# OCR-D/ocrd_keraslm

Measured on AMD Instinct MI355X. Metric: chars/sec training (stacked-LSTM forward+backward+Adam), higher is better.
Workload: dtype bf16; 1 GPU; cfg2: depth=2 width=512 length=256 V=256 1 context, stateful training, 3072 streams/GPU, synthetic 10M-char corpus (SURVEY.md 8d); streams_per_gpu=3072, global_batch=3072, seq_len=256, parallelism=dp1

## Files before the change

ocrd_keraslm_amd/csrc/api.hip:

```cpp
#include <hip/hip_runtime.h>
#include <stdio.h>
#include <stdlib.h>
#include <string.h>
#include <time.h>

#include <functional>
#include <utility>

#include <vector>

#include "kl_common.h"
#include "kl_kernels.h"

namespace {

inline size_t align_up(size_t x, size_t a) { return (x + a - 1) / a * a; }
inline int round_up_i(int x, int a) { return (x + a - 1) / a * a; }

struct Carver {
  unsigned char* base;
  size_t off = 0;
  explicit Carver(void* b) : base(reinterpret_cast<unsigned char*>(b)) {}
  template <typename T>
  T* take(size_t count) {
// ... 23 lines not shown
  unsigned* scan_flags = nullptr;
};

struct WindowWs {
  float* P1;
  std::vector<void*> H;
  std::vector<float*> C;
  float* logits;
  float* rowstat;
  int *s_idx, *s_ctx, *s_tgt;
  int* ids_tm = nullptr;
  int scan2_rows = 0;
  bool scan2_bwd = false;
  float *s_masks, *s_probs;
  unsigned *scan_cnt, *scan_status;
  float* reg_scratch;
  std::vector<bf16_t*> G, dZ, Hd;
  std::vector<bf16_t*> Cb;
  std::vector<bf16_t*> Xhi, Xlo;
  std::vector<bf16_t*> HTf, HdT;
  bool ht_ready = false;
  bool km_plan = false;
  bf16_t *dZT, *HT, *dlogits, *dlogitsT, *OHT, *dEKT_bf, *dEK_bf;
  std::vector<bf16_t*> OHC;
  float *dH, *dEKT;
  std::vector<float*> dc0, dc1, dCtxKT;
};

}

struct kl_handle {
  kl_config cfg;
  int Vp;
  size_t n_params;
  std::vector<size_t> off_K, off_U, off_b, off_Ctx;
  size_t off_E;
  float* params = nullptr;
  void* derived_ws = nullptr;
  size_t derived_bytes = 0;
  Derived d;
  int precision = 0;
  struct GraphKey {
    int kind, B, T, flags, precision;
    const void *states, *loss_acc, *ws, *grads;
    int layout = 0;
    bool operator==(const GraphKey& o) const {
// ... 35 lines not shown
  int inc_small_min = KL_SMALL_STEP_N;
  bool scan2 = true;
  int scan2_rows = 0;
  int scan2_pf = -1;
  bool scan2_bf16 = true;
  bool logits_ws = true;
  bool proj_ws = true;
  bool w128 = true;
  bool w128_tables = true;
  bool w128_multi = true;
  bool w128_fuse = true;
  int w128_min = 1;
  bool fwd8 = true;
  bool fwd8_all = false;
  bool fwd8_tab = true;
  bool fwd8_ls = true;
  bool fwd8_local = true;
  int fwd8_pf = -1;
  bool rt_local = true;
  bool regtile = true;
  bool scan2_flags = true;
  bool flags_zeroed = false;
  bool fuse_wg = true;
  int scan2_pfb = -1;
  int wide_fwd_min = 96;
  double trace_flops[2] = {0.0, 0.0};
  bool trace_on = false;
  std::vector<std::pair<hipEvent_t, hipEvent_t>> trace_ev[2];
  size_t trace_used[2] = {0, 0};
  bool trace_open[2] = {false, false};
  bool trace_persistent[2] = {false, false};
  const char* trace_name[2] = {"lstm_fwd_step_kernel", "lstm_bwd_step_kernel"};
  void trace_begin(int kind, hipStream_t s) {
    if (!trace_on) return;
    if (trace_used[kind] == trace_ev[kind].size()) {
      hipEvent_t a, b;
      if (hipEventCreate(&a) != hipSuccess || hipEventCreate(&b) != hipSuccess) { trace_on = false; return; }
      trace_ev[kind].emplace_back(a, b);
    }
    (void)hipEventRecord(trace_ev[kind][trace_used[kind]].first, s);
    trace_open[kind] = true;
  }
  void trace_end(int kind, hipStream_t s) {
    if (!trace_on || !trace_open[kind]) return;
    trace_open[kind] = false;
    (void)hipEventRecord(trace_ev[kind][trace_used[kind]].second, s);
// ... 132 lines not shown
  if (training) {
    o.G.assign(L, nullptr); o.dZ.assign(L, nullptr); o.Hd.assign(L, nullptr); o.Cb.assign(L, nullptr);
    o.dc0.assign(L, nullptr); o.dc1.assign(L, nullptr);
    for (size_t l = 0; l < L; ++l) {
      o.G[l] = cv.take<bf16_t>(BT * 4 * W);
      o.dZ[l] = cv.take<bf16_t>(BT * 4 * W);
      o.Hd[l] = l > 0 ? cv.take<bf16_t>(BT * W) : nullptr;
      o.Cb[l] = cv.take<bf16_t>((BT + B) * W);
      o.dc0[l] = cv.take<float>((size_t)B * W);
      o.dc1[l] = cv.take<float>((size_t)B * W);
    }
    o.dZT = cv.take<bf16_t>(4 * W * BTp);
    o.HT = cv.take<bf16_t>(W * BTp);
    o.ids_tm = cv.take<int>((BT + B) * 2);
    o.HTf.assign(L, nullptr); o.HdT.assign(L, nullptr);
    if ((B & 7) == 0) {
      for (size_t l = 0; l < L; ++l) {
        o.HTf[l] = cv.take<bf16_t>(W * (BT + B));
        o.HdT[l] = l > 0 ? cv.take<bf16_t>(W * BT) : nullptr;
      }
    }
    o.dlogits = cv.take<bf16_t>(BT * Vp);
    o.dlogitsT = cv.take<bf16_t>(Vp * BTp);
    o.OHT = cv.take<bf16_t>(Vp * BTp);
    o.OHC.assign(c.n_ctx, nullptr);
    o.dCtxKT.assign(c.n_ctx, nullptr);
    for (int n = 0; n < c.n_ctx; ++n) {
      o.OHC[n] = cv.take<bf16_t>((size_t)c.ctx_vocab * BTp);
      o.dCtxKT[n] = cv.take<float>(4 * W * (size_t)c.ctx_vocab);
    }
    o.dH = cv.take<float>(BT * W);
    o.dEKT = cv.take<float>(4 * W * Vp);
    o.dEKT_bf = cv.take<bf16_t>(4 * W * Vp);
    o.dEK_bf = cv.take<bf16_t>(Vp * 4 * W);
  }
  return align_up(cv.off, 256);
}

#define KL_TRY(expr)            \
  do {                          \
    int _e = (expr);            \
    if (_e != 0) return _e;     \
  } while (0)

int hip_ok(hipError_t e) { return e == hipSuccess ? 0 : KL_ERR_LAUNCH; }

int prepare_impl(kl_handle* h, int precision, hipStream_t s) {
  const kl_config& c = h->cfg;
  const int W = c.width, V = c.voc_size, Vp = h->Vp;
  const float* P = h->params;
  Derived& d = h->d;
  const bool split = precision == KL_PREC_SPLIT;
  if (!h->flags_zeroed) {
    hipStreamCaptureStatus cap = hipStreamCaptureStatusNone;
    if (hipStreamIsCapturing(s, &cap) == hipSuccess && cap == hipStreamCaptureStatusNone) {
      KL_TRY(kl_zero_async(d.scan_flags, (size_t)(KL_SCAN_FLAGS + 64) * sizeof(unsigned), s));
      h->flags_zeroed = true;
    }
  }
  const float* E = P + h->off_E;
// ... 129 lines not shown
      KlScanFwdWide a;
      memset(&a, 0, sizeof(a));
      a.B = B; a.T = T; a.W = W;
      a.UT = d.UT_hi[l];
      const bool v2 = w.scan2_rows != 0;
      const bool f8_tab = v2 && l == 0 && h->fwd8 && h->fwd8_tab && !h->fwd8_all && d.comb != nullptr && c.n_ctx == 1 && w.scan2_rows == 32 &&
                          h->scan2_bf16 && h->sentinel_roll && T >= 3 && h->fwd8_ls;
      const bool f8 = v2 && h->fwd8 && w.scan2_rows == 32 && h->scan2_bf16 && h->sentinel_roll && T >= 3 &&
                      (l > 0 || c.n_ctx > 1 || h->fwd8_all || f8_tab);
      if (l > 0) {
        const bool masked_in = masks != nullptr && (l - 1) > 0;
        const bf16_t* X = masked_in ? w.Hd[l - 1] : (const bf16_t*)w.H[l - 1] + BW;
        int pe = KL_ERR_SHAPE;
        if (v2 && h->scan2_bf16 && h->proj_ws)
          pe = kl_launch_proj_ws(X, d.KTp[l], d.bp[l], reinterpret_cast<bf16_t*>(w.P1), (long)B * T, W, w.scan_status, s);
        if (pe == KL_ERR_SHAPE)
          pe = kl_launch_gemm_tn(X, v2 ? d.KTp[l] : d.KT_hi[l], w.P1, v2 ? d.bp[l] : P + h->off_b[l], B * T, 4 * W, W, W, W, 4 * W,
                                 v2 && h->scan2_bf16 ? 1 : 0, 1, 1.f, s);
        KL_TRY(pe);
        a.P = w.P1;
        a.p_bf16 = v2 && h->scan2_bf16 ? 1 : 0;
      } else if (f8_tab) {
        KL_TRY(kl_launch_comb_table(d.EKp, d.CtxKp[0], c.voc_size, c.ctx_vocab, 4 * W, d.comb, s));
        KL_TRY(kl_launch_rows_tm(idx, ctx, c.n_ctx, B, T, c.ctx_vocab, w.ids_tm, s));
        a.P = reinterpret_cast<const float*>(d.comb);
        a.p_bf16 = 1;
        a.ids_tm = w.ids_tm;
        a.V = c.voc_size; a.ctx_vocab = c.ctx_vocab;
      } else if (v2 && (c.n_ctx > 1 || f8)) {
        KL_TRY(kl_launch_p_gather_il(d.EKp, d.CtxKp.data(), c.n_ctx, idx, ctx, B, T, W, c.voc_size, c.ctx_vocab,
                                     reinterpret_cast<bf16_t*>(w.P1), s));
        a.P = w.P1;
        a.p_bf16 = 1;
      } else if (v2) {
        KL_TRY(kl_launch_ids_tm(idx, ctx, c.n_ctx, B, T, W, c.voc_size, c.ctx_vocab, w.ids_tm, s));
        a.EK = d.EKp;
        a.CtxK[0] = c.n_ctx > 0 ? d.CtxKp[0] : nullptr;
        a.n_ctx = c.n_ctx;
        a.ids_tm = w.ids_tm;
        a.V = c.voc_size; a.ctx_vocab = c.ctx_vocab;
      } else {
        a.EK = d.EK;
        for (int n = 0; n < c.n_ctx; ++n) a.CtxK[n] = d.CtxK[n];
        a.n_ctx = c.n_ctx;
        a.idx = idx; a.ctx = ctx;
        a.bias = P + h->off_b[0];
      }
// ... 519 lines not shown
  const char* env8t = getenv("KL_W128_TABLES");
  if (env8t) h->w128_tables = atoi(env8t) != 0;
  const char* env8mm = getenv("KL_W128_MULTI");
  if (env8mm) h->w128_multi = atoi(env8mm) != 0;
  const char* env8q = getenv("KL_W128_MIN");
  if (env8q) h->w128_min = atoi(env8q);
  const char* env8m = getenv("KL_FWD8");
  if (env8m) { h->fwd8 = atoi(env8m) != 0; h->fwd8_all = atoi(env8m) == 2; }
  const char* env8r = getenv("KL_FWD8_LS");
  if (env8r) h->fwd8_ls = atoi(env8r) != 0;
  const char* env8n = getenv("KL_FWD8_LOCAL");
  if (env8n) h->fwd8_local = atoi(env8n) != 0;
  const char* env8o = getenv("KL_FWD8_PF");
  if (env8o) h->fwd8_pf = atoi(env8o);
  const char* env8l = getenv("KL_RT_LOCAL");
  if (env8l) h->rt_local = atoi(env8l) != 0;
  const char* env8k = getenv("KL_REGTILE");
  if (env8k) h->regtile = atoi(env8k) != 0;
  const char* env8g = getenv("KL_SCAN2_FLAGS");
  if (env8g) h->scan2_flags = atoi(env8g) != 0;
  h->flags_zeroed = false;
  const char* env8f = getenv("KL_FUSE_WG");
  if (env8f) h->fuse_wg = atoi(env8f) != 0;
  const char* env8d = getenv("KL_SCAN2_PFB");
  if (env8d) h->scan2_pfb = atoi(env8d);
  const char* env5 = getenv("KL_WIDE_FWD_MIN");
  if (env5) h->wide_fwd_min = atoi(env5);
  return kl_zero_page_ready();
}

int kl_prepare(kl_handle* h, int precision, void* stream) {
  if (!h) return KL_ERR_ARG;
  if (!h->params) return KL_ERR_STATE;
  if (precision != KL_PREC_BF16 && precision != KL_PREC_SPLIT) return KL_ERR_ARG;
  return prepare_impl(h, precision, (hipStream_t)stream);
}

size_t kl_window_workspace_bytes(const kl_handle* h, int B, int T, int training) {
  if (!h || B < 1 || T < 1) return 0;
  return carve_window(h, nullptr, B, T, training, nullptr);
}

static int forward_window_body(kl_handle* h, int B, int T, const int32_t* idx, const int32_t* ctx, const int32_t* tgt,
                      float* states, float* probs, float* loss_acc, void* ws, size_t ws_bytes, void* stream) {
  if (!h || !idx || !states || !ws || B < 1 || T < 1) return KL_ERR_ARG;
  if (h->cfg.n_ctx > 0 && !ctx) return KL_ERR_ARG;
// ... 122 lines not shown
    } else if (dz_km) {
      KL_TRY(kl_launch_gemm_an(w.dZ[l], (const bf16_t*)w.H[l], grads + h->off_U[l], 4 * W, W, BT, 4 * W, W, 4 * W, 1, s, 1));
    } else if (w.ht_ready) {
      KL_TRY(kl_launch_gemm_tn(w.HTf[l], w.dZT, grads + h->off_U[l], nullptr, W, 4 * W, BT, ldtf, BTp, 4 * W, 2, ksplit, 1.f, s));
    } else {
      KL_TRY(kl_launch_transpose_bf16((const bf16_t*)w.H[l], W, w.HT, BTp, BT, W, s));
      KL_TRY(kl_launch_gemm_tn(w.HT, w.dZT, grads + h->off_U[l], nullptr, W, 4 * W, BTp, BTp, BTp, 4 * W, 2, ksplit, 1.f, s));
    }
    if (!db_done) KL_TRY(kl_launch_colsum_bf16(w.dZ[l], 4 * W, BT, 4 * W, grads + h->off_b[l], s));
    if (l > 0) {
      const bool masked_in = masks != nullptr && (l - 1) > 0;
      const bf16_t* X = masked_in ? w.Hd[l - 1] : (const bf16_t*)w.H[l - 1] + BW;
      if (pair_uk) {
      } else if (dz_km) {
        KL_TRY(kl_launch_gemm_an(w.dZ[l], X, grads + h->off_K[l], 4 * W, W, BT, 4 * W, W, 4 * W, 1, s, 1));
      } else if (w.ht_ready) {
        const bf16_t* XT = masked_in ? w.HdT[l - 1] : w.HTf[l - 1] + B;
        KL_TRY(kl_launch_gemm_tn(XT, w.dZT, grads + h->off_K[l], nullptr, W, 4 * W, BT, masked_in ? (long)BT : ldtf, BTp, 4 * W, 2, ksplit, 1.f, s));
      } else {
        KL_TRY(kl_launch_transpose_bf16(X, W, w.HT, BTp, BT, W, s));
        KL_TRY(kl_launch_gemm_tn(w.HT, w.dZT, grads + h->off_K[l], nullptr, W, 4 * W, BTp, BTp, BTp, 4 * W, 2, ksplit, 1.f, s));
      }
    } else {
      if (kl_launch_onehot_dense(idx, B, T, Vp, 0, 1, w.OHT, BTp, s) == KL_ERR_SHAPE) {
        KL_TRY(kl_zero_async(w.OHT, (size_t)Vp * BTp * sizeof(bf16_t), s));
        KL_TRY(kl_launch_onehot_t(idx, B, T, V, 0, 1, w.OHT, BTp, s));
      }
      KL_TRY(kl_zero_async(w.dEKT, (size_t)4 * W * Vp * sizeof(float), s));
      bool pair_ctx = dz_km && h->fuse_wg && c.n_ctx >= 1 && (Vp % 128) == 0 &&
                      kl_gemm_an_applicable(4 * W, Vp + c.ctx_vocab, BT, 4 * W);
      if (pair_ctx) {
        if (kl_launch_onehot_dense(ctx, B, T, c.ctx_vocab, 0, c.n_ctx, w.OHC[0], BTp, s) == KL_ERR_SHAPE) {
          KL_TRY(kl_zero_async(w.OHC[0], (size_t)c.ctx_vocab * BTp * sizeof(bf16_t), s));
          KL_TRY(kl_launch_onehot_t(ctx, B, T, c.ctx_vocab, 0, c.n_ctx, w.OHC[0], BTp, s));
        }
        KL_TRY(kl_zero_async(w.dCtxKT[0], (size_t)4 * W * c.ctx_vocab * sizeof(float), s));
        const int pe = kl_launch_gemm_an2(w.dZ[l], w.OHT, w.dEKT, 4 * W, Vp, BT, 4 * W, BTp, Vp, 0,
                                          w.OHC[0], w.dCtxKT[0], c.ctx_vocab, BTp, c.ctx_vocab, 0, s, 0);
        if (pe == KL_ERR_SHAPE) pair_ctx = false;
        else KL_TRY(pe);
      }
      if (pair_ctx) {
      } else if (dz_km) KL_TRY(kl_launch_gemm_an(w.dZ[l], w.OHT, w.dEKT, 4 * W, Vp, BT, 4 * W, BTp, Vp, 0, s));
      else KL_TRY(kl_launch_gemm_tn(w.dZT, w.OHT, w.dEKT, nullptr, 4 * W, Vp, BTp, BTp, BTp, Vp, 2, ksplit, 1.f, s));
      KL_TRY(kl_launch_f32_to_bf16_t(w.dEKT, Vp, 4 * W, Vp, w.dEKT_bf, nullptr, Vp, 0, s));
      KL_TRY(kl_launch_f32_to_bf16_t(w.dEKT, Vp, 4 * W, Vp, w.dEK_bf, nullptr, 4 * W, 1, s));
      KL_TRY(kl_launch_gemm_tn(d.ET, w.dEKT_bf, grads + h->off_K[0], nullptr, W, 4 * W, Vp, Vp, Vp, 4 * W, 0, 1, 1.f, s));
      KL_TRY(kl_launch_gemm_tn(w.dEK_bf, d.Kn[0], grads + h->off_E, nullptr, V, W, 4 * W, 4 * W, 4 * W, W, 2, 1, 1.f, s));
      for (int n = 0; n < c.n_ctx; ++n) {
        if (!(pair_ctx && n == 0)) {
          if (kl_launch_onehot_dense(ctx, B, T, c.ctx_vocab, n, c.n_ctx, w.OHC[n], BTp, s) == KL_ERR_SHAPE) {
            KL_TRY(kl_zero_async(w.OHC[n], (size_t)c.ctx_vocab * BTp * sizeof(bf16_t), s));
            KL_TRY(kl_launch_onehot_t(ctx, B, T, c.ctx_vocab, n, c.n_ctx, w.OHC[n], BTp, s));
          }
          KL_TRY(kl_zero_async(w.dCtxKT[n], (size_t)4 * W * c.ctx_vocab * sizeof(float), s));
          if (dz_km) KL_TRY(kl_launch_gemm_an(w.dZ[l], w.OHC[n], w.dCtxKT[n], 4 * W, c.ctx_vocab, BT, 4 * W, BTp, c.ctx_vocab, 0, s));
          else KL_TRY(kl_launch_gemm_tn(w.dZT, w.OHC[n], w.dCtxKT[n], nullptr, 4 * W, c.ctx_vocab, BTp, BTp, BTp,
                                        c.ctx_vocab, 2, ksplit, 1.f, s));
        }
        const size_t krow = (size_t)(W + n * c.ctx_dim) * 4 * W;
        KL_TRY(kl_launch_ctx_grads(P + h->off_Ctx[n], P + h->off_K[0] + krow, 4 * W, c.ctx_vocab, c.ctx_dim,
                                   w.dCtxKT[n], c.ctx_vocab, 4 * W, grads + h->off_K[0] + krow, 4 * W,
                                   grads + h->off_Ctx[n], s));
      }
    }
      return 0;
  };
  bool bscanned = false;
  const int n_rb_all = (B + 15) / 16, nug = W / 16;
  const bool thin_fits = (n_rb_all + 512 / nug - 1) / (512 / nug) <= (W == 1024 ? 8 : 4) &&
                         (long)T * B * 4 * W * 2 <= 0xfffffff0L;
  const bool wide_fits = h->wide_bwd && kl_scan_bwd_wide_applicable(B, T, W) && BTp == BT && (B & 7) == 0;
  const bool seq128 = h->scan_enabled && h->seq_bwd && h->w128 && B >= h->w128_min && kl_scan_w128_applicable(B, T, W) && !w.scan2_bwd;
// ... 720 lines not shown
```

ocrd_keraslm_amd/csrc/elementwise.hip:

```cpp
#include <string.h>

#include "kl_common.h"
#include "kl_kernels.h"

namespace {

struct CtxTabs { const float* t[8]; };

__global__ void embed_gather_kernel(const float* __restrict__ E, CtxTabs tabs, int n_ctx, int ctx_dim, int W,
                                    const int* __restrict__ idx, const int* __restrict__ ctx, int B, int T,
                                    bf16_t* __restrict__ X, long ldx, int Dp) {
  const int chunks = Dp >> 3;
  const long total = (long)B * T * chunks;
  for (long e = blockIdx.x * (long)blockDim.x + threadIdx.x; e < total; e += (long)gridDim.x * blockDim.x) {
    const int c = (int)(e % chunks);
    const long row = e / chunks;
    const int b = (int)(row % B), t = (int)(row / B);
    const int id = idx[(long)b * T + t];
    frag16 o;
#pragma unroll
    for (int j = 0; j < 8; ++j) {
      const int d = c * 8 + j;
      float v = 0.f;
      if (d < W) {
// ... 453 lines not shown
    gx = max(gx, (jobs[j].cols + 63) / 64);
    gy = max(gy, (all.job[j].rows_pad + 63) / 64);
  }
  hipLaunchKernelGGL(f32_to_bf16_jobs_kernel, dim3(gx, gy, n), dim3(256), 0, stream, all);
  return ok();
}

__global__ void comb_table_kernel(const float* __restrict__ A, const float* __restrict__ B, int R2, int N8, bf16_t* __restrict__ out, long total) {
  for (long e = blockIdx.x * (long)blockDim.x + threadIdx.x; e < total; e += (long)gridDim.x * blockDim.x) {
    const int j = (int)(e % N8);
    const long row = e / N8;
    const int c = (int)(row % R2), v = (int)(row / R2);
    const float4* pa = reinterpret_cast<const float4*>(A + ((long)v * N8 + j) * 8);
    const float4* pb = reinterpret_cast<const float4*>(B + ((long)c * N8 + j) * 8);
    const float4 a0 = pa[0], a1 = pa[1], b0 = pb[0], b1 = pb[1];
    uint4 o;
    o.x = (unsigned)f2bf(a0.x + b0.x) | ((unsigned)f2bf(a0.y + b0.y) << 16);
    o.y = (unsigned)f2bf(a0.z + b0.z) | ((unsigned)f2bf(a0.w + b0.w) << 16);
    o.z = (unsigned)f2bf(a1.x + b1.x) | ((unsigned)f2bf(a1.y + b1.y) << 16);
    o.w = (unsigned)f2bf(a1.z + b1.z) | ((unsigned)f2bf(a1.w + b1.w) << 16);
    reinterpret_cast<uint4*>(out)[e] = o;
  }
}
__global__ void rows_tm_kernel(const int* __restrict__ idx, const int* __restrict__ ctx, int n_ctx, int Bn, int T, int R2, int* __restrict__ out) {
  const long total = (long)Bn * T;
  for (long e = blockIdx.x * (long)blockDim.x + threadIdx.x; e < total; e += (long)gridDim.x * blockDim.x) {
    const int b = (int)(e % Bn), t = (int)(e / Bn);
    const long src = (long)b * T + t;
    out[e] = idx[src] * R2 + (n_ctx > 0 ? ctx[src * n_ctx] : 0);
  }
}

int kl_launch_comb_table(const float* A, const float* B, int R1, int R2, int N, bf16_t* out, hipStream_t stream) {
  if ((N & 7) || R1 < 1 || R2 < 1) return KL_ERR_SHAPE;
  const long total = (long)R1 * R2 * (N / 8);
  hipLaunchKernelGGL(comb_table_kernel, dim3(grid_for(total, 256)), dim3(256), 0, stream, A, B, R2, N / 8, out, total);
  return ok();
}
int kl_launch_rows_tm(const int* idx, const int* ctx, int n_ctx, int Bn, int T, int R2, int* out, hipStream_t stream) {
  hipLaunchKernelGGL(rows_tm_kernel, dim3(grid_for((long)Bn * T, 256)), dim3(256), 0, stream, idx, ctx, n_ctx, Bn, T, R2, out);
  return ok();
}

int kl_launch_softmax_ce(float* logits, long ld, int rows, int V, const int* tgt, int B, int T, float inv_count,
                         bf16_t* dlogits, long ld_dl, float* loss_acc, float* rowstat, int time_major,
                         hipStream_t stream, int last_only) {
  dim3 grid((rows + 3) / 4);
  const bool stats = tgt != nullptr && loss_acc != nullptr && rowstat != nullptr;
  const bool one_pass = V <= 256 && (V & 3) == 0 && (ld & 3) == 0 && (!dlogits || ((ld_dl & 3) == 0 && ld_dl <= 256));
  if (one_pass)
    hipLaunchKernelGGL(softmax_ce_v256_kernel, grid, dim3(256), 0, stream, logits, ld, rows, V, tgt, B, T, inv_count,
                       dlogits, ld_dl, stats ? rowstat : nullptr, time_major, last_only);
  else
    hipLaunchKernelGGL(softmax_ce_kernel, grid, dim3(256), 0, stream, logits, ld, rows, V, tgt, B, T, inv_count,
                       dlogits, ld_dl, stats ? rowstat : nullptr, time_major, last_only);
  if (stats) {
    int nb = (rows + 4095) / 4096;
    if (nb > 64) nb = 64;
    hipLaunchKernelGGL(rowstat_reduce_kernel, dim3(nb), dim3(256), 0, stream, rowstat, rows, loss_acc);
  }
  return ok();
}

// ... 132 lines not shown
```

ocrd_keraslm_amd/csrc/kl_kernels.h:

```cpp
#pragma once
#include <hip/hip_runtime.h>
#include <stdint.h>

#include "keraslm_hip.h"

typedef unsigned short bf16_t;

#include <atomic>
#include <mutex>
#define KL_MAX_DEVICES 64
struct KlLdsGrant {
  std::atomic<size_t> granted[KL_MAX_DEVICES];
  std::mutex slow;
};
static inline int kl_grant_lds(KlLdsGrant& g, const void* fn, size_t lds) {
  int dev = 0;
  if (hipGetDevice(&dev) != hipSuccess) return KL_ERR_LAUNCH;
  if (dev < 0 || dev >= KL_MAX_DEVICES)
    return hipFuncSetAttribute(fn, hipFuncAttributeMaxDynamicSharedMemorySize, (int)lds) == hipSuccess ? 0 : KL_ERR_LAUNCH;
  if (lds <= g.granted[dev].load(std::memory_order_acquire)) return 0;
  std::lock_guard<std::mutex> lock(g.slow);
  if (lds <= g.granted[dev].load(std::memory_order_relaxed)) return 0;
  if (hipFuncSetAttribute(fn, hipFuncAttributeMaxDynamicSharedMemorySize, (int)lds) != hipSuccess) return KL_ERR_LAUNCH;
  g.granted[dev].store(lds, std::memory_order_release);
// ... 193 lines not shown
int kl_launch_dh_ws(const bf16_t* dlogits, const bf16_t* ET, bf16_t* dH, long M, int W, int Vp, hipStream_t stream);
int kl_launch_logits_ce_w128(const bf16_t* X, const bf16_t* E, const bf16_t* ET, const int* tgt, bf16_t* dlogits, float* dH, float* rowstat, int B,
                             int T, int W, int V, int Vp, float inv_count, int last_only, hipStream_t stream);
int kl_launch_rowstat_reduce(const float* rowstat, int rows, float* loss_acc, hipStream_t stream);
int kl_launch_proj_ws(const bf16_t* X, const bf16_t* KTp, const float* bp, bf16_t* P, long M, int W, unsigned* status,
                      hipStream_t stream);

int kl_launch_thin_gemm(const KlOperand* op, int M, int N, float* C, long ldc, const float* bias, int split,
                        hipStream_t stream);

int kl_launch_embed_gather(const float* E, const float* const* ctx_tabs, int n_ctx, int ctx_dim, int W,
                           const int* idx, const int* ctx, int B, int T, bf16_t* X, long ldx, int Dp,
                           hipStream_t stream);
int kl_launch_transpose_bf16(const bf16_t* in, long ld_in, bf16_t* out, long ld_out, int rows, int cols,
                             hipStream_t stream);
#define KL_CONV_MAX_JOBS 24
struct KlConvJob {
  const float* in; long ld_in; int rows, cols, rows_pad, transpose;
  bf16_t* out_hi; bf16_t* out_lo; long ld_out;
};
struct KlConvJobs { KlConvJob job[KL_CONV_MAX_JOBS]; };
int kl_launch_f32_to_bf16_jobs(const KlConvJob* jobs, int n, hipStream_t stream);
int kl_launch_comb_table(const float* A, const float* B, int R1, int R2, int N, bf16_t* out, hipStream_t stream);
int kl_launch_rows_tm(const int* idx, const int* ctx, int n_ctx, int Bn, int T, int R2, int* out, hipStream_t stream);
int kl_launch_f32_to_bf16_t(const float* in, long ld_in, int rows, int cols, bf16_t* out_hi, bf16_t* out_lo,
                            long ld_out, int transpose, hipStream_t stream);
int kl_launch_softmax_ce(float* logits, long ld, int rows, int V, const int* tgt, int B, int T, float inv_count,
                         bf16_t* dlogits, long ld_dl, float* loss_acc, float* rowstat, int time_major,
                         hipStream_t stream, int last_only = 0);
int kl_launch_adam(float* p, const float* g, float* m, float* v, size_t n, float lr_t, float b1, float b2,
                   float eps, float clip, float grad_scale, hipStream_t stream);
int kl_launch_onehot_t(const int* ids, int B, int T, int n_classes, int col, int n_cols, bf16_t* out, long ld,
                       hipStream_t stream);
int kl_launch_onehot_dense(const int* ids, int B, int T, int n_rows, int col, int n_cols, bf16_t* out, long ld,
                           hipStream_t stream);
int kl_launch_regulariser_grads(const float* E, int V, int W, const float* const* ctx_tabs, int n_ctx, int ctx_vocab,
                                int ctx_dim, float* gE, float* const* gCtx, float* loss_acc, float* scratch,
                                hipStream_t stream);
int kl_launch_state_to_rows(const float* states, int B, int W, int L, int layer, bf16_t* h_bf16, float* h_f32,
                            float* c_f32, hipStream_t stream);
int kl_launch_fill_f32(float* p, size_t n, float v, hipStream_t stream);
int kl_launch_fill_bf16(bf16_t* p, size_t n, unsigned short bits, hipStream_t stream);
int kl_zero_async(void* p, size_t bytes, hipStream_t stream);
int kl_fill_u32_async(void* p, size_t bytes, unsigned value, hipStream_t stream);
int kl_zero_coherent_async(unsigned* p, size_t n_words, hipStream_t stream);

int kl_launch_small_table(const float* A, int R, int D, const float* Kmat, long ldk, int N, float* C, long ldc,
                          hipStream_t stream);
int kl_launch_p1_gather(const float* EK, const float* const* ctxk, int n_ctx, const float* bias, const int* idx,
                        const int* ctx, int B, int T, int N, float* P, hipStream_t stream);
int kl_launch_colsum_bf16(const bf16_t* in, long ld, int rows, int cols, float* out, hipStream_t stream);
int kl_launch_rows_to_state(const void* h_rows, int h_is_f32, const float* c_rows, int B, int W, int L, int layer,
                            float* states, hipStream_t stream);
int kl_launch_ctx_grads(const float* Ctx, const float* K0rows, long ldk, int R, int D, const float* dT, long ldt, int N,
                        float* gK, long ldg, float* gCtx, hipStream_t stream);
int kl_launch_rows_tm_to_bm(const float* in, long ld_in, float* out, int B, int T, int V, hipStream_t stream);

#define KL_SMALL_STEP_N 16
struct KlIncCellArgs {
  int n, W, split;
  float* pool; long slot_ld;
  const int* slot_in; const int* slot_out;
  int h_off, c_off, x_off;
  const bf16_t* UF; const bf16_t* KF;
  const float* T1; const int* i1; const float* T2; const int* i2; const float* bias;
};
#define KL_HOST_STEP_MAX 256
struct KlHostIdx {
  int slot_in[KL_HOST_STEP_MAX];
  int slot_out[KL_HOST_STEP_MAX];
  unsigned short idx[KL_HOST_STEP_MAX];
  unsigned short ctx[KL_HOST_STEP_MAX];
};
struct KlHostTargets { unsigned short t[KL_HOST_STEP_MAX]; };
struct KlStepFinish {
  int n, V, W;
  const float* logits; long ld;
  int softmax, by_target, head_k;
  const int* target;
  const float* pool; long slot_ld; const int* slot_out;
// ... 18 lines not shown
```

Before: 33.93 million chars/s.

## Replace one-hot GEMM embedding gradients with radix-sort segmented sums

Computes the layer-0 embedding and context table gradients by radix-sorting the (char, ctx) keys, summing dZ rows per key in segments, and then forming marginals. This replaces the one-hot construction and the dense one-hot GEMMs over BT. Its workspace overlays the one-hot buffers. The path adds several small kernel launches, including a single-block scan, and relies on enough rows per key to pay off. Index clamping is also added to rows_tm.

```diff
diff --git a/ocrd_keraslm_amd/csrc/api.hip b/ocrd_keraslm_amd/csrc/api.hip
--- a/ocrd_keraslm_amd/csrc/api.hip
+++ b/ocrd_keraslm_amd/csrc/api.hip
@@ -69,6 +69,7 @@
   bool ht_ready = false;
   bool km_plan = false;
   bf16_t *dZT, *HT, *dlogits, *dlogitsT, *OHT, *dEKT_bf, *dEK_bf;
+  size_t tg_bytes = 0;
   std::vector<bf16_t*> OHC;
   float *dH, *dEKT;
   std::vector<float*> dc0, dc1, dCtxKT;
@@ -150,6 +151,8 @@
   bool scan2_flags = true;
   bool flags_zeroed = false;
   bool fuse_wg = true;
+  bool table_segsum = true;
+  unsigned long long table_segsum_windows = 0;
   int scan2_pfb = -1;
   int wide_fwd_min = 96;
   double trace_flops[2] = {0.0, 0.0};
@@ -328,11 +331,18 @@
     }
     o.dlogits = cv.take<bf16_t>(BT * Vp);
     o.dlogitsT = cv.take<bf16_t>(Vp * BTp);
+    o.tg_bytes = 0;
+    if (h->table_segsum && c.n_ctx <= 1 && kl_table_segsum_pays(c.n_ctx, B, T, (int)V, c.ctx_vocab))
+      o.tg_bytes = kl_table_segsum_ws_bytes(c.n_ctx, B, T, (int)V, c.ctx_vocab, (int)W);
+    cv.off = align_up(cv.off, 256);
+    const size_t oh_begin = cv.off;
     o.OHT = cv.take<bf16_t>(Vp * BTp);
     o.OHC.assign(c.n_ctx, nullptr);
     o.dCtxKT.assign(c.n_ctx, nullptr);
+    if (c.n_ctx > 0) o.OHC[0] = cv.take<bf16_t>((size_t)c.ctx_vocab * BTp);
+    if (cv.off < oh_begin + o.tg_bytes) cv.off = oh_begin + o.tg_bytes;
     for (int n = 0; n < c.n_ctx; ++n) {
-      o.OHC[n] = cv.take<bf16_t>((size_t)c.ctx_vocab * BTp);
+      if (n > 0) o.OHC[n] = cv.take<bf16_t>((size_t)c.ctx_vocab * BTp);
       o.dCtxKT[n] = cv.take<float>(4 * W * (size_t)c.ctx_vocab);
     }
     o.dH = cv.take<float>(BT * W);
@@ -342,6 +352,17 @@
   }
   return align_up(cv.off, 256);
 }
+
+}
+
+extern "C" size_t kl_test_table_segsum_bytes(const kl_handle* h, int B, int T) {
+  WindowWs w;
+  carve_window(h, nullptr, B, T, 1, &w);
+  return w.tg_bytes;
+}
+extern "C" unsigned long long kl_test_table_segsum_windows(const kl_handle* h) { return h->table_segsum_windows; }
+
+namespace {
 
 #define KL_TRY(expr)            \
   do {                          \
@@ -517,7 +538,7 @@
         a.p_bf16 = v2 && h->scan2_bf16 ? 1 : 0;
       } else if (f8_tab) {
         KL_TRY(kl_launch_comb_table(d.EKp, d.CtxKp[0], c.voc_size, c.ctx_vocab, 4 * W, d.comb, s));
-        KL_TRY(kl_launch_rows_tm(idx, ctx, c.n_ctx, B, T, c.ctx_vocab, w.ids_tm, s));
+        KL_TRY(kl_launch_rows_tm(idx, ctx, c.n_ctx, B, T, c.voc_size, c.ctx_vocab, w.ids_tm, s));
         a.P = reinterpret_cast<const float*>(d.comb);
         a.p_bf16 = 1;
         a.ids_tm = w.ids_tm;
@@ -1083,6 +1104,8 @@
   h->flags_zeroed = false;
   const char* env8f = getenv("KL_FUSE_WG");
   if (env8f) h->fuse_wg = atoi(env8f) != 0;
+  const char* env_tsum = getenv("KL_TABLE_SEGSUM");
+  if (env_tsum) h->table_segsum = atoi(env_tsum) != 0;
   const char* env8d = getenv("KL_SCAN2_PFB");
   if (env8d) h->scan2_pfb = atoi(env8d);
   const char* env5 = getenv("KL_WIDE_FWD_MIN");
@@ -1251,12 +1274,21 @@
         KL_TRY(kl_launch_gemm_tn(w.HT, w.dZT, grads + h->off_K[l], nullptr, W, 4 * W, BTp, BTp, BTp, 4 * W, 2, ksplit, 1.f, s));
       }
     } else {
-      if (kl_launch_onehot_dense(idx, B, T, Vp, 0, 1, w.OHT, BTp, s) == KL_ERR_SHAPE) {
-        KL_TRY(kl_zero_async(w.OHT, (size_t)Vp * BTp * sizeof(bf16_t), s));
-        KL_TRY(kl_launch_onehot_t(idx, B, T, V, 0, 1, w.OHT, BTp, s));
-      }
-      KL_TRY(kl_zero_async(w.dEKT, (size_t)4 * W * Vp * sizeof(float), s));
-      bool pair_ctx = dz_km && h->fuse_wg && c.n_ctx >= 1 && (Vp % 128) == 0 &&
+      bool segsum = false;
+      if (w.tg_bytes > 0) {
+        KL_TRY(kl_launch_table_grads(w.dZ[l], idx, ctx, c.n_ctx, B, T, V, Vp, c.ctx_vocab, W, w.dEKT,
+                                     c.n_ctx == 1 ? w.dCtxKT[0] : nullptr, w.OHT, w.tg_bytes, s));
+        segsum = true;
+        ++h->table_segsum_windows;
+      }
+      if (!segsum) {
+        if (kl_launch_onehot_dense(idx, B, T, Vp, 0, 1, w.OHT, BTp, s) == KL_ERR_SHAPE) {
+          KL_TRY(kl_zero_async(w.OHT, (size_t)Vp * BTp * sizeof(bf16_t), s));
+          KL_TRY(kl_launch_onehot_t(idx, B, T, V, 0, 1, w.OHT, BTp, s));
+        }
+        KL_TRY(kl_zero_async(w.dEKT, (size_t)4 * W * Vp * sizeof(float), s));
+      }
+      bool pair_ctx = !segsum && dz_km && h->fuse_wg && c.n_ctx >= 1 && (Vp % 128) == 0 &&
                       kl_gemm_an_applicable(4 * W, Vp + c.ctx_vocab, BT, 4 * W);
       if (pair_ctx) {
         if (kl_launch_onehot_dense(ctx, B, T, c.ctx_vocab, 0, c.n_ctx, w.OHC[0], BTp, s) == KL_ERR_SHAPE) {
@@ -1269,7 +1301,7 @@
         if (pe == KL_ERR_SHAPE) pair_ctx = false;
         else KL_TRY(pe);
       }
-      if (pair_ctx) {
+      if (pair_ctx || segsum) {
       } else if (dz_km) KL_TRY(kl_launch_gemm_an(w.dZ[l], w.OHT, w.dEKT, 4 * W, Vp, BT, 4 * W, BTp, Vp, 0, s));
       else KL_TRY(kl_launch_gemm_tn(w.dZT, w.OHT, w.dEKT, nullptr, 4 * W, Vp, BTp, BTp, BTp, Vp, 2, ksplit, 1.f, s));
       KL_TRY(kl_launch_f32_to_bf16_t(w.dEKT, Vp, 4 * W, Vp, w.dEKT_bf, nullptr, Vp, 0, s));
@@ -1277,7 +1309,7 @@
       KL_TRY(kl_launch_gemm_tn(d.ET, w.dEKT_bf, grads + h->off_K[0], nullptr, W, 4 * W, Vp, Vp, Vp, 4 * W, 0, 1, 1.f, s));
       KL_TRY(kl_launch_gemm_tn(w.dEK_bf, d.Kn[0], grads + h->off_E, nullptr, V, W, 4 * W, 4 * W, 4 * W, W, 2, 1, 1.f, s));
       for (int n = 0; n < c.n_ctx; ++n) {
-        if (!(pair_ctx && n == 0)) {
+        if (!((pair_ctx || segsum) && n == 0)) {
           if (kl_launch_onehot_dense(ctx, B, T, c.ctx_vocab, n, c.n_ctx, w.OHC[n], BTp, s) == KL_ERR_SHAPE) {
             KL_TRY(kl_zero_async(w.OHC[n], (size_t)c.ctx_vocab * BTp * sizeof(bf16_t), s));
             KL_TRY(kl_launch_onehot_t(ctx, B, T, c.ctx_vocab, n, c.n_ctx, w.OHC[n], BTp, s));
diff --git a/ocrd_keraslm_amd/csrc/elementwise.hip b/ocrd_keraslm_amd/csrc/elementwise.hip
--- a/ocrd_keraslm_amd/csrc/elementwise.hip
+++ b/ocrd_keraslm_amd/csrc/elementwise.hip
@@ -499,12 +499,17 @@
     reinterpret_cast<uint4*>(out)[e] = o;
   }
 }
-__global__ void rows_tm_kernel(const int* __restrict__ idx, const int* __restrict__ ctx, int n_ctx, int Bn, int T, int R2, int* __restrict__ out) {
+__global__ void rows_tm_kernel(const int* __restrict__ idx, const int* __restrict__ ctx, int n_ctx, int Bn, int T, int V, int R2,
+                               int* __restrict__ out) {
   const long total = (long)Bn * T;
   for (long e = blockIdx.x * (long)blockDim.x + threadIdx.x; e < total; e += (long)gridDim.x * blockDim.x) {
     const int b = (int)(e % Bn), t = (int)(e / Bn);
     const long src = (long)b * T + t;
-    out[e] = idx[src] * R2 + (n_ctx > 0 ? ctx[src * n_ctx] : 0);
+    int id = idx[src];
+    id = id < 0 ? 0 : (id >= V ? V - 1 : id);
+    int c = n_ctx > 0 ? ctx[src * n_ctx] : 0;
+    c = c < 0 ? 0 : (c >= R2 ? R2 - 1 : c);
+    out[e] = id * R2 + c;
   }
 }
 
@@ -514,8 +519,8 @@
   hipLaunchKernelGGL(comb_table_kernel, dim3(grid_for(total, 256)), dim3(256), 0, stream, A, B, R2, N / 8, out, total);
   return ok();
 }
-int kl_launch_rows_tm(const int* idx, const int* ctx, int n_ctx, int Bn, int T, int R2, int* out, hipStream_t stream) {
-  hipLaunchKernelGGL(rows_tm_kernel, dim3(grid_for((long)Bn * T, 256)), dim3(256), 0, stream, idx, ctx, n_ctx, Bn, T, R2, out);
+int kl_launch_rows_tm(const int* idx, const int* ctx, int n_ctx, int Bn, int T, int V, int R2, int* out, hipStream_t stream) {
+  hipLaunchKernelGGL(rows_tm_kernel, dim3(grid_for((long)Bn * T, 256)), dim3(256), 0, stream, idx, ctx, n_ctx, Bn, T, V, R2, out);
   return ok();
 }
 
diff --git a/ocrd_keraslm_amd/csrc/kl_kernels.h b/ocrd_keraslm_amd/csrc/kl_kernels.h
--- a/ocrd_keraslm_amd/csrc/kl_kernels.h
+++ b/ocrd_keraslm_amd/csrc/kl_kernels.h
@@ -239,7 +239,7 @@
 struct KlConvJobs { KlConvJob job[KL_CONV_MAX_JOBS]; };
 int kl_launch_f32_to_bf16_jobs(const KlConvJob* jobs, int n, hipStream_t stream);
 int kl_launch_comb_table(const float* A, const float* B, int R1, int R2, int N, bf16_t* out, hipStream_t stream);
-int kl_launch_rows_tm(const int* idx, const int* ctx, int n_ctx, int Bn, int T, int R2, int* out, hipStream_t stream);
+int kl_launch_rows_tm(const int* idx, const int* ctx, int n_ctx, int Bn, int T, int V, int R2, int* out, hipStream_t stream);
 int kl_launch_f32_to_bf16_t(const float* in, long ld_in, int rows, int cols, bf16_t* out_hi, bf16_t* out_lo,
                             long ld_out, int transpose, hipStream_t stream);
 int kl_launch_softmax_ce(float* logits, long ld, int rows, int V, const int* tgt, int B, int T, float inv_count,
@@ -273,6 +273,11 @@
                         float* gK, long ldg, float* gCtx, hipStream_t stream);
 int kl_launch_rows_tm_to_bm(const float* in, long ld_in, float* out, int B, int T, int V, hipStream_t stream);
 
+size_t kl_table_segsum_ws_bytes(int n_ctx, int B, int T, int V, int ctx_vocab, int W);
+bool kl_table_segsum_pays(int n_ctx, int B, int T, int V, int ctx_vocab);
+int kl_launch_table_grads(const bf16_t* dZ, const int* idx, const int* ctx, int n_ctx, int B, int T, int V, int Vp,
+                          int ctx_vocab, int W, float* dEKT, float* dCtxT, void* ws, size_t ws_bytes, hipStream_t stream);
+
 #define KL_SMALL_STEP_N 16
 struct KlIncCellArgs {
   int n, W, split;
diff --git a/ocrd_keraslm_amd/csrc/table_grads.hip b/ocrd_keraslm_amd/csrc/table_grads.hip
--- /dev/null
+++ b/ocrd_keraslm_amd/csrc/table_grads.hip
@@ -0,0 +1,403 @@
+#include "kl_common.h"
+#include "kl_kernels.h"
+
+namespace {
+
+constexpr int KL_TG_TILE = 4096;
+constexpr int KL_TG_WIN = 512;
+
+inline int ok() { return hipGetLastError() == hipSuccess ? 0 : KL_ERR_LAUNCH; }
+
+struct TgSrc {
+  const int* idx;
+  const int* ctx;
+  int n_ctx, B, T, V, ctx_vocab, R2, nkeys;
+};
+__device__ __forceinline__ int tg_key(const TgSrc& s, long r) {
+  const int b = (int)(r % s.B), t = (int)(r / s.B);
+  const long src = (long)b * s.T + t;
+  int v = s.idx[src];
+  const bool v_out = v < 0 || v >= s.V;
+  if (s.n_ctx == 0) return v_out ? s.nkeys : v;
+  int c = s.ctx[src * s.n_ctx];
+  const bool c_out = c < 0 || c >= s.ctx_vocab;
+  if (v_out && c_out) return s.nkeys;
+  if (v_out) v = s.V;
+  if (c_out) c = s.ctx_vocab;
+  return v * s.R2 + c;
+}
+
+__global__ __launch_bounds__(256) void tg_count_kernel(TgSrc s, const int* __restrict__ key_in, long n, int shift, int nb,
+                                                       int* __restrict__ hist, int* __restrict__ present, int n_present) {
+  __shared__ int h[256];
+  h[threadIdx.x] = 0;
+  if (present)
+    for (long i = (long)blockIdx.x * 256 + threadIdx.x; i < n_present; i += (long)gridDim.x * 256) present[i] = 0;
+  __syncthreads();
+  const long r0 = (long)blockIdx.x * KL_TG_TILE;
+  for (int i = threadIdx.x; i < KL_TG_TILE; i += 256) {
+    const long r = r0 + i;
+    if (r < n) atomicAdd(&h[((key_in ? key_in[r] : tg_key(s, r)) >> shift) & 255], 1);
+  }
+  __syncthreads();
+  hist[threadIdx.x * nb + blockIdx.x] = h[threadIdx.x];
+}
+
+__global__ __launch_bounds__(1024) void tg_scan_kernel(int* __restrict__ a, int n) {
+  __shared__ int buf[16 * 1024];
+  __shared__ int wsum[16];
+  const int tid = threadIdx.x, wave = tid >> 6, lane = tid & 63;
+  int carry = 0;
+  for (int c0 = 0; c0 < n; c0 += 16 * 1024) {
+    const int m = min(16 * 1024, n - c0);
+#pragma unroll
+    for (int j = 0; j < 16; ++j) {
+      const int i = j * 1024 + tid;
+      buf[i] = i < m ? a[c0 + i] : 0;
+    }
+    __syncthreads();
+    int v[16], sum = 0;
+#pragma unroll
+    for (int j = 0; j < 16; ++j) {
+      v[j] = buf[tid * 16 + j];
+      sum += v[j];
+    }
+    int x = sum;
+#pragma unroll
+    for (int o = 1; o < 64; o <<= 1) {
+      const int y = __shfl_up(x, o, 64);
+      if (lane >= o) x += y;
+    }
+    if (lane == 63) wsum[wave] = x;
+    __syncthreads();
+    int before = carry, total = 0;
+#pragma unroll
+    for (int w = 0; w < 16; ++w) {
+      before += w < wave ? wsum[w] : 0;
+      total += wsum[w];
+    }
+    int run = before + x - sum;
+#pragma unroll
+    for (int j = 0; j < 16; ++j) {
+      buf[tid * 16 + j] = run;
+      run += v[j];
+    }
+    __syncthreads();
+#pragma unroll
+    for (int j = 0; j < 16; ++j) {
+      const int i = j * 1024 + tid;
+      if (i < m) a[c0 + i] = buf[i];
+    }
+    carry += total;
+    __syncthreads();
+  }
+}
+
+__global__ __launch_bounds__(256) void tg_scatter_kernel(TgSrc s, const int* __restrict__ key_in, const int* __restrict__ row_in,
+                                                         long n, int shift, int nb, const int* __restrict__ hist,
+                                                         int* __restrict__ key_out, int* __restrict__ row_out) {
+  __shared__ int base[256];
+  __shared__ int cnt[4][256];
+  const int tid = threadIdx.x, wave = tid >> 6, lane = tid & 63;
+  base[tid] = hist[tid * nb + blockIdx.x];
+  cnt[0][tid] = cnt[1][tid] = cnt[2][tid] = cnt[3][tid] = 0;
+  __syncthreads();
+  const unsigned long long below = (1ull << lane) - 1ull;
+  const long r0 = (long)blockIdx.x * KL_TG_TILE;
+  for (int it = 0; it < KL_TG_TILE / 256 && r0 + it * 256 < n; ++it) {
+    const long r = r0 + it * 256 + tid;
+    const bool valid = r < n;
+    int k = 0, row = 0;
+    if (valid) {
+      k = key_in ? key_in[r] : tg_key(s, r);
+      row = row_in ? row_in[r] : (int)r;
+    }
+    const int d = (k >> shift) & 255;
+    unsigned long long m = __ballot(valid);
+#pragma unroll
+    for (int bit = 0; bit < 8; ++bit) {
+      const unsigned long long bb = __ballot((d >> bit) & 1);
+      m &= ((d >> bit) & 1) ? bb : ~bb;
+    }
+    const int rank = __popcll(m & below);
+    if (valid && rank == 0) cnt[wave][d] = __popcll(m);
+    __syncthreads();
+    if (valid) {
+      int pos = base[d] + rank;
+      for (int w = 0; w < wave; ++w) pos += cnt[w][d];
+      key_out[pos] = k;
+      row_out[pos] = row;
+    }
+    __syncthreads();
+    base[tid] += cnt[0][tid] + cnt[1][tid] + cnt[2][tid] + cnt[3][tid];
+    cnt[0][tid] = cnt[1][tid] = cnt[2][tid] = cnt[3][tid] = 0;
+    __syncthreads();
+  }
+}
+
+template <int NJ>
+__global__ __launch_bounds__(256) void tg_segsum_kernel(const bf16_t* __restrict__ dZ, const int* __restrict__ skey,
+                                                        const int* __restrict__ srow, long n, int nkeys,
+                                                        float* __restrict__ comb, float* __restrict__ part,
+                                                        int* __restrict__ present) {
+  constexpr int NC = NJ * 512;
+  constexpr int RF = NJ >= 8 ? 2 : (NJ >= 4 ? 4 : 8);
+  __shared__ int lk[4][KL_TG_WIN], lr[4][KL_TG_WIN];
+  const int wave = threadIdx.x >> 6, lane = threadIdx.x & 63;
+  const long w = (long)blockIdx.x * 4 + wave;
+  const long p0 = w * KL_TG_WIN;
+  const int cntw = p0 < n ? (int)min((long)KL_TG_WIN, n - p0) : 0;
+  int pe = 0;
+  for (int j = lane; j < KL_TG_WIN; j += 64) {
+    int k = nkeys, rr = 0;
+    if (j < cntw) {
+      k = skey[p0 + j];
+      rr = srow[p0 + j];
+    }
+    lk[wave][j] = k;
+    lr[wave][j] = rr;
+    pe += __popcll(__ballot(k < nkeys));
+  }
+  __syncthreads();
+  if (pe == 0) return;
+  const int prev_key = p0 > 0 ? skey[p0 - 1] : -1;
+  const int next_key = (pe == KL_TG_WIN && p0 + KL_TG_WIN < n) ? skey[p0 + KL_TG_WIN] : -1;
+
+  const uint4* zb = reinterpret_cast<const uint4*>(dZ);
+  float acc[NJ * 8];
+#pragma unroll
+  for (int e = 0; e < NJ * 8; ++e) acc[e] = 0.f;
+  int cur = __builtin_amdgcn_readfirstlane(lk[wave][0]);
+  bool first = true;
+
+  auto flush = [&](bool last) {
+    float* dst;
+    if (first && prev_key == cur) {
+      dst = part + (w * 2) * NC;
+    } else {
+      if (lane == 0) present[cur] = 1;
+      dst = (last && next_key == cur) ? part + (w * 2 + 1) * NC : comb + (long)cur * NC;
+    }
+#pragma unroll
+    for (int j = 0; j < NJ; ++j) {
+      float4* o = reinterpret_cast<float4*>(dst + j * 512 + lane * 8);
+      o[0] = make_float4(acc[j * 8 + 0], acc[j * 8 + 1], acc[j * 8 + 2], acc[j * 8 + 3]);
+      o[1] = make_float4(acc[j * 8 + 4], acc[j * 8 + 5], acc[j * 8 + 6], acc[j * 8 + 7]);
+    }
+  };
+  auto load = [&](uint4 (&buf)[RF][NJ], int q) {
+#pragma unroll
+    for (int i = 0; i < RF; ++i) {
+      const long row = __builtin_amdgcn_readfirstlane(lr[wave][min(q + i, KL_TG_WIN - 1)]);
+#pragma unroll
+      for (int j = 0; j < NJ; ++j) buf[i][j] = zb[row * (NJ * 64) + j * 64 + lane];
+    }
+  };
+  auto consume = [&](const uint4 (&buf)[RF][NJ], int q) {
+#pragma unroll
+    for (int i = 0; i < RF; ++i) {
+      if (q + i < pe) {
+        const int k = __builtin_amdgcn_readfirstlane(lk[wave][q + i]);
+        if (k != cur) {
+          flush(false);
+          first = false;
+          cur = k;
+#pragma unroll
+          for (int e = 0; e < NJ * 8; ++e) acc[e] = 0.f;
+        }
+#pragma unroll
+        for (int j = 0; j < NJ; ++j) {
+          const unsigned x[4] = {buf[i][j].x, buf[i][j].y, buf[i][j].z, buf[i][j].w};
+#pragma unroll
+          for (int h = 0; h < 4; ++h) {
+            acc[j * 8 + 2 * h] += __builtin_bit_cast(float, x[h] << 16);
+            acc[j * 8 + 2 * h + 1] += __builtin_bit_cast(float, x[h] & 0xffff0000u);
+          }
+        }
+      }
+    }
+  };
+  uint4 ba[RF][NJ], bb[RF][NJ];
+  load(ba, 0);
+  for (int q = 0; q < pe; q += 2 * RF) {
+    load(bb, q + RF);
+    consume(ba, q);
+    load(ba, q + 2 * RF);
+    consume(bb, q + RF);
+  }
+  flush(true);
+}
+
+__global__ __launch_bounds__(256) void tg_fixup_kernel(const int* __restrict__ skey, long n, int nkeys, int nc,
+                                                       float* __restrict__ comb, const float* __restrict__ part) {
+  __shared__ int first_end;
+  const long w = blockIdx.x;
+  const long p0 = w * KL_TG_WIN, p1 = min(n, p0 + KL_TG_WIN);
+  const int kl = skey[p1 - 1];
+  if (kl >= nkeys || p1 >= n || skey[p1] != kl) return;
+  if (p0 > 0 && skey[p0 - 1] == kl && skey[p0] == kl) return;
+  long m = 0;
+  for (long w0 = w + 1;; w0 += 256) {
+    if (threadIdx.x == 0) first_end = 256;
+    __syncthreads();
+    const long e = min(n, (w0 + threadIdx.x + 1) * KL_TG_WIN);
+    if (w0 + threadIdx.x < (n + KL_TG_WIN - 1) / KL_TG_WIN && (e >= n || skey[e] != kl)) atomicMin(&first_end, (int)threadIdx.x);
+    __syncthreads();
+    const int fe = first_end;
+    __syncthreads();
+    if (fe < 256) {
+      m = w0 + fe - w;
+      break;
+    }
+  }
+  for (int g = threadIdx.x * 4; g < nc; g += 1024) {
+    f32x4 a = *reinterpret_cast<const f32x4*>(part + (w * 2 + 1) * nc + g);
+#pragma unroll 8
+    for (long i = 1; i <= m; ++i) a += *reinterpret_cast<const f32x4*>(part + ((w + i) * 2) * nc + g);
+    *reinterpret_cast<f32x4*>(comb + (long)kl * nc + g) = a;
+  }
+}
+
+__global__ __launch_bounds__(256) void tg_marginals_kernel(const float* __restrict__ comb, const int* __restrict__ present, int nc,
+                                                           int V, int nv, int Vp, int R2, int cv, float* __restrict__ dEKT,
+                                                           float* __restrict__ dCtxT) {
+  __shared__ int list[256];
+  __shared__ int wcnt[4];
+  const int tid = threadIdx.x, wave = tid >> 6, lane = tid & 63;
+  const bool is_e = (int)blockIdx.x < Vp;
+  const int v = blockIdx.x, c = blockIdx.x - Vp;
+  const int n_cand = is_e ? (v < V ? R2 : 0) : nv;
+  const int g = (blockIdx.y * 256 + tid) * 4;
+  f32x4 a = {0.f, 0.f, 0.f, 0.f};
+  for (int i0 = 0; i0 < n_cand; i0 += 256) {
+    const int i = i0 + tid;
+    const int k = is_e ? v * R2 + i : i * R2 + c;
+    const bool p = i < n_cand && present[k] != 0;
+    const unsigned long long b = __ballot(p);
+    if (lane == 0) wcnt[wave] = __popcll(b);
+    __syncthreads();
+    int pos = __popcll(b & ((1ull << lane) - 1ull));
+    for (int ww = 0; ww < wave; ++ww) pos += wcnt[ww];
+    const int cnt = wcnt[0] + wcnt[1] + wcnt[2] + wcnt[3];
+    if (p) list[pos] = k;
+    __syncthreads();
+    if (g < nc) {
+      int j = 0;
+      for (; j + 8 <= cnt; j += 8) {
+        f32x4 x[8];
+#pragma unroll
+        for (int u = 0; u < 8; ++u) x[u] = *reinterpret_cast<const f32x4*>(comb + (long)list[j + u] * nc + g);
+#pragma unroll
+        for (int u = 0; u < 8; ++u) a += x[u];
+      }
+      for (; j < cnt; ++j) a += *reinterpret_cast<const f32x4*>(comb + (long)list[j] * nc + g);
+    }
+    __syncthreads();
+  }
+  if (g >= nc) return;
+  if (is_e) {
+#pragma unroll
+    for (int e = 0; e < 4; ++e) dEKT[(long)(g + e) * Vp + v] = a[e];
+  } else {
+#pragma unroll
+    for (int e = 0; e < 4; ++e) dCtxT[(long)(g + e) * cv + c] = a[e];
+  }
+}
+
+inline size_t tg_align(size_t x) { return (x + 255) & ~(size_t)255; }
+
+struct TgPlan {
+  long n, nwin;
+  int nb, nkeys, nv, R2, nc, passes;
+  size_t o_comb, o_k0, o_r0, o_k1, o_r1, o_hist, o_present, o_part, bytes;
+};
+
+bool tg_plan(int n_ctx, int B, int T, int V, int ctx_vocab, int W, TgPlan& p) {
+  if (n_ctx < 0 || n_ctx > 1 || B < 1 || T < 1 || V < 1 || ctx_vocab < 0) return false;
+  if (W != 128 && W != 256 && W != 512 && W != 1024) return false;
+  p.n = (long)B * T;
+  if (p.n >= (1L << 31)) return false;
+  p.R2 = n_ctx > 0 ? ctx_vocab + 1 : 1;
+  p.nv = n_ctx > 0 ? V + 1 : V;
+  const long nk = (long)p.nv * p.R2;
+  if (nk >= (1L << 24)) return false;
+  p.nkeys = (int)nk;
+  p.nc = 4 * W;
+  p.nb = (int)((p.n + KL_TG_TILE - 1) / KL_TG_TILE);
+  p.nwin = (p.n + KL_TG_WIN - 1) / KL_TG_WIN;
+  const int nbits = 32 - __builtin_clz((unsigned)p.nkeys);
+  p.passes = (nbits + 7) / 8;
+  size_t off = 0;
+  p.o_comb = off; off = tg_align(off + (size_t)p.nkeys * p.nc * sizeof(float));
+  p.o_k0 = off;   off = tg_align(off + (size_t)p.n * sizeof(int));
+  p.o_r0 = off;   off = tg_align(off + (size_t)p.n * sizeof(int));
+  p.o_k1 = off;   off = tg_align(off + (size_t)p.n * sizeof(int));
+  p.o_r1 = off;   off = tg_align(off + (size_t)p.n * sizeof(int));
+  p.o_hist = off; off = tg_align(off + (size_t)256 * p.nb * sizeof(int));
+  p.o_present = off; off = tg_align(off + (size_t)p.nkeys * sizeof(int));
+  p.o_part = off; off = tg_align(off + (size_t)p.nwin * 2 * p.nc * sizeof(float));
+  p.bytes = off;
+  return true;
+}
+
+}
+
+size_t kl_table_segsum_ws_bytes(int n_ctx, int B, int T, int V, int ctx_vocab, int W) {
+  TgPlan p;
+  return tg_plan(n_ctx, B, T, V, ctx_vocab, W, p) ? p.bytes : 0;
+}
+
+int kl_launch_table_grads(const bf16_t* dZ, const int* idx, const int* ctx, int n_ctx, int B, int T, int V, int Vp,
+                          int ctx_vocab, int W, float* dEKT, float* dCtxT, void* ws, size_t ws_bytes, hipStream_t stream) {
+  TgPlan p;
+  if (!tg_plan(n_ctx, B, T, V, ctx_vocab, W, p) || p.bytes > ws_bytes || Vp < V) return KL_ERR_SHAPE;
+  if (!dZ || !idx || (n_ctx > 0 && (!ctx || !dCtxT)) || !dEKT || !ws || ((size_t)ws & 255) || ((size_t)dZ & 15)) return KL_ERR_ARG;
+  unsigned char* base = reinterpret_cast<unsigned char*>(ws);
+  float* comb = reinterpret_cast<float*>(base + p.o_comb);
+  int* kbuf[2] = {reinterpret_cast<int*>(base + p.o_k0), reinterpret_cast<int*>(base + p.o_k1)};
+  int* rbuf[2] = {reinterpret_cast<int*>(base + p.o_r0), reinterpret_cast<int*>(base + p.o_r1)};
+  int* hist = reinterpret_cast<int*>(base + p.o_hist);
+  int* present = reinterpret_cast<int*>(base + p.o_present);
+  float* part = reinterpret_cast<float*>(base + p.o_part);
+  TgSrc s;
+  s.idx = idx; s.ctx = ctx; s.n_ctx = n_ctx; s.B = B; s.T = T; s.V = V; s.ctx_vocab = ctx_vocab; s.R2 = p.R2; s.nkeys = p.nkeys;
+
+  const int* kin = nullptr;
+  const int* rin = nullptr;
+  for (int pass = 0; pass < p.passes; ++pass) {
+    int* kout = kbuf[pass & 1];
+    int* rout = rbuf[pass & 1];
+    hipLaunchKernelGGL(tg_count_kernel, dim3(p.nb), dim3(256), 0, stream, s, kin, p.n, 8 * pass, p.nb, hist,
+                       pass == 0 ? present : nullptr, p.nkeys);
+    hipLaunchKernelGGL(tg_scan_kernel, dim3(1), dim3(1024), 0, stream, hist, 256 * p.nb);
+    hipLaunchKernelGGL(tg_scatter_kernel, dim3(p.nb), dim3(256), 0, stream, s, kin, rin, p.n, 8 * pass, p.nb, hist, kout, rout);
+    kin = kout;
+    rin = rout;
+  }
+  const dim3 gs((unsigned)((p.nwin + 3) / 4));
+  switch (W) {
+    case 128: hipLaunchKernelGGL(tg_segsum_kernel<1>, gs, dim3(256), 0, stream, dZ, kin, rin, p.n, p.nkeys, comb, part, present); break;
+    case 256: hipLaunchKernelGGL(tg_segsum_kernel<2>, gs, dim3(256), 0, stream, dZ, kin, rin, p.n, p.nkeys, comb, part, present); break;
+    case 512: hipLaunchKernelGGL(tg_segsum_kernel<4>, gs, dim3(256), 0, stream, dZ, kin, rin, p.n, p.nkeys, comb, part, present); break;
+    default: hipLaunchKernelGGL(tg_segsum_kernel<8>, gs, dim3(256), 0, stream, dZ, kin, rin, p.n, p.nkeys, comb, part, present); break;
+  }
+  hipLaunchKernelGGL(tg_fixup_kernel, dim3((unsigned)p.nwin), dim3(256), 0, stream, kin, p.n, p.nkeys, p.nc, comb, part);
+  const int cv = n_ctx > 0 ? ctx_vocab : 0;
+  hipLaunchKernelGGL(tg_marginals_kernel, dim3((unsigned)(Vp + cv), (unsigned)((p.nc / 4 + 255) / 256)), dim3(256), 0, stream,
+                     comb, present, p.nc, V, p.nv, Vp, p.R2, cv, dEKT, dCtxT);
+  return ok();
+}
+
+bool kl_table_segsum_pays(int n_ctx, int B, int T, int V, int ctx_vocab) {
+  const long nkeys = (long)(n_ctx > 0 ? V + 1 : V) * (n_ctx > 0 ? ctx_vocab + 1 : 1);
+  return (long)B * T >= 8 * nkeys;
+}
+
+extern "C" size_t kl_test_table_segsum_ws_bytes(int n_ctx, int B, int T, int V, int ctx_vocab, int W) {
+  return kl_table_segsum_ws_bytes(n_ctx, B, T, V, ctx_vocab, W);
+}
+extern "C" int kl_test_table_grads(const void* dZ, const int* idx, const int* ctx, int n_ctx, int B, int T, int V, int Vp,
+                                   int ctx_vocab, int W, float* dEKT, float* dCtxT, void* ws, size_t ws_bytes, void* stream) {
+  return kl_launch_table_grads(reinterpret_cast<const bf16_t*>(dZ), idx, ctx, n_ctx, B, T, V, Vp, ctx_vocab, W, dEKT, dCtxT, ws,
+                               ws_bytes, reinterpret_cast<hipStream_t>(stream));
+}
```

Result: no change. 34.25 million chars/s (median of 6 runs) (+0.9%).
